# wrchen530/batrack

Hardware: AMD Instinct MI355X
Metric: BA iterations/s on 64-KF/128k-edge graph (higher is better)
Workload: dtype f32

## Files before the change

### batrack_amd/csrc/ba_plan.hpp

```cpp
#pragma once
#include <array>
#include <atomic>
#include <chrono>
#include <cstddef>
#include <cstdio>
#include <cstdint>
#include <string>
#include <vector>

#include "../../include/batrack_ba.h"

namespace bt {

constexpr int kLanes = 64;
constexpr int kTileCamSoft = 16;
constexpr int kTileCamHard = 64;
constexpr int kTileCamF64 = 32;
constexpr int kFewHubs = 64;
constexpr int kMaxFree = 255;
constexpr int kMaxFreeWide = 2048;
constexpr int kPairAccStride = 32;
constexpr int kPrivY = 16, kPrivP = 4;
constexpr int kPrivArrive = 8192;
constexpr int kPairGeomFloats = 20;
constexpr int kLdsRowStride = 66;
constexpr int kMaxLevelCols = 4;
constexpr size_t kLdsBudget = 160 * 1024 - 512;
inline size_t solve_lds_bytes_raw(size_t nnzb, size_t D, size_t nupd, size_t n, size_t nlev, size_t ndp, size_t elem) {
    size_t b = (nnzb * 36 + 2 * D) * elem;
    b = (b + 15) / 16 * 16;
    b += nupd * 3 * sizeof(unsigned short);
    b = (b + 15) / 16 * 16;
    b += (nnzb + 4 * (n + 1) + nlev + 1 + n + ndp) * sizeof(int);
    b = (b + 15) / 16 * 16 + nlev * kMaxLevelCols * 8 * sizeof(int);
    return b + 64;
}
constexpr int kSpGroupMax = 32;
constexpr int kMaxTilePairs = 192;

#ifdef __HIPCC__
#define BT_HD __host__ __device__
#else
#define BT_HD
#endif
BT_HD inline size_t priv_copy_doubles(size_t D, size_t pairs) { return (size_t)kPrivY * D + (size_t)kPrivP * pairs * kPairAccStride; }
BT_HD inline size_t priv_doubles(size_t D, size_t pairs) { return priv_copy_doubles(D, pairs) + kPrivArrive / 2; }
BT_HD inline size_t sp_tile_doubles(int max_rows16, int max_tile_pairs) {
    const size_t nt = (size_t)max_rows16 / 16;
    return nt * (nt + 1) / 2 * 256 + (size_t)max_rows16 + (size_t)(max_tile_pairs > 0 ? max_tile_pairs : 1) * 32;
}

constexpr size_t kEtileLdsBudget = 160 * 1024 - 512;
BT_HD inline size_t etile_full_lds_bytes(int max_rows16, int max_tile_pairs, size_t rsz) {
    const size_t mtp = (size_t)(max_tile_pairs > 0 ? max_tile_pairs : 1), rows = (size_t)max_rows16;
    size_t smax = 1;
    while (smax < mtp) smax <<= 1;
    return (size_t)4 * 26 * smax * sizeof(double) + (rows * kLdsRowStride + 128 + mtp * kPairGeomFloats) * rsz + rows * sizeof(int) + 64;
}

struct Route {
    enum : int { kTile = 0, kStream = 1, kEdge = 2, kEtile = 3 };
    enum : int { kSolveLds = 0, kSolveLds32 = 1, kSolveGlobal = 2, kSolveDense = 3, kSolveFused = 4, kSolvePipe = 5 };
    int kernel;
    int prec;
    int wide;
    int solver;
    int fuse_update;
    int upd_wgs;
};

struct PlanDev {
    int E, n_buf, p_tot, fixedp, n_all, n, D, m, P, T, slots, erows, nnzb, nupd, max_rows16;
    const int32_t *kx;
    const uint32_t *act_bits;
    const int32_t *act_rank;
    const int32_t *pair_i, *pair_j;
    const int32_t *tile_trk0, *tile_ntrk, *tile_ncam, *tile_cam0, *tile_slot0, *tile_nslot, *tile_erow0;
    const int32_t *tile_cams;
    const int32_t *slot_edge, *slot_pair;
    const uint16_t *slot_lab;
    const int32_t *tile_pair0, *tile_npair, *tile_pairs;
    const uint16_t *tile_cut8, *tile_cut16;
    const int32_t *tile_ij, *tile_kx;
    const int32_t *tile_flags;
    const uint8_t *slot_lp;
    int max_tile_pairs, max_tile_slots, max_cams;
    long long e_all;
    const uint16_t *slot_code;
    const uint8_t *tile_la;
    const int32_t *tile_rec;
    const int32_t *it_edge;
    const uint32_t *tile_sinfo;
    const int32_t *pm_edge, *pm_rec;
    const uint8_t *pm_lb, *pm_la;
    const int32_t *pp_ptr, *pp_idx;
    const int32_t *sg_ptr; int sg_n;
    int et_lgts;
    int sp_ok;
    int pm_ok;
    const int32_t *lz_trk, *lz_ptr, *lz_edge, *lz_pair;
    int nlz;
    int dev_id;
    int wide;
    int trk_off;
    int em_self;
    int em_ok, em_its, em_lgs;
    int st_ok;
    int st_min, em_min;
    const int32_t *col_ptr, *row_idx, *upd_ptr, *upd, *blk_col, *upd_next;
    int nlev, ndp;
    const int32_t *perm, *blk_src, *lvl_ptr, *lvl_cols, *col_lvl, *dp_ptr, *dp;
    const int32_t *fz_pend_ptr, *fz_pend, *fz_lazy_ptr, *fz_lazy, *fz_yurg, *fz_meta, *fz_pmeta, *bs_sync, *fz_rowinfo, *fz_pfirst, *fz_psecond;
    int fz_npend, fz_nlazy, fz_ok;
    int fzp_ok;
    const int32_t *lvl_meta;
    Route route;
};

constexpr size_t kStatusBytes = 1024;
constexpr int kStatusHandoff = 2;

struct WsLayout {
    size_t sys, pairacc, zero_bytes;
    size_t packed, pairgeo, qw, lfac, linv, zvec, dx, dx0, dxg, status, spart, esave, total;
    size_t priv;
};

// ... 162 lines not shown
```

### batrack_amd/csrc/ba_plan_solver.cpp

```cpp
#include "ba_plan.hpp"

#include <algorithm>
#include <numeric>

namespace bt {
namespace {

using Pattern = std::vector<std::vector<uint8_t>>;

void couple_all(Pattern &nz, std::vector<int32_t> &cset) {
    std::sort(cset.begin(), cset.end());
    cset.erase(std::unique(cset.begin(), cset.end()), cset.end());
    for (size_t u = 0; u < cset.size(); ++u)
        for (size_t v = 0; v <= u; ++v) nz[(size_t)cset[u]][(size_t)cset[v]] = 1;
}

int system_pattern(const bt_plan *pl, bool sharded, const DevPlanStats *dstats, const uint64_t *pk, int64_t E, Pattern &nz) {
    const int64_t n = pl->info.n, fixedp = pl->info.fixedp, p_tot = pl->info.p_tot;
    nz.assign((size_t)n, std::vector<uint8_t>((size_t)n, 0));
    for (int64_t c = 0; c < n; ++c) nz[(size_t)c][(size_t)c] = 1;
    for (int64_t t = 0; t < pl->info.tiles && !sharded; ++t) {
        const int32_t c0 = pl->tile_cam0[(size_t)t], nc = pl->tile_ncam[(size_t)t];
        for (int32_t u = 0; u < nc; ++u)
            for (int32_t v = 0; v <= u; ++v)
// ... 224 lines not shown
            for (int pass = 0; pass < 2; ++pass)
                for (int32_t q = pl->lvl_ptr[(size_t)l]; q < pl->lvl_ptr[(size_t)l + 1]; ++q) {
                    const int32_t j = pl->lvl_cols[(size_t)q];
                    for (int32_t b = pl->col_ptr[(size_t)j] + 1; b < pl->col_ptr[(size_t)j + 1]; ++b) {
                        const int32_t r = pl->row_idx[(size_t)b];
                        if (pass == 0) { if (seen[(size_t)r] != l) { seen[(size_t)r] = l; cnt[(size_t)r] = 0; } cnt[(size_t)r]++; }
                        else if (cnt[(size_t)r] > 1) pl->blk_col[(size_t)b] |= 1 << 16;
                    }
                }
        }
    }
    pl->dp_ptr.assign((size_t)n + 1, 0);
    pl->dp.clear();
    for (int64_t j = 0; j < n; ++j) {
        pl->dp_ptr[(size_t)j] = (int32_t)pl->dp.size();
        pl->dp.insert(pl->dp.end(), dplist[(size_t)j].begin(), dplist[(size_t)j].end());
    }
    pl->dp_ptr[(size_t)n] = (int32_t)pl->dp.size();

    pl->lvl_meta.assign((size_t)nlev * kMaxLevelCols * 8, 0);
    for (int32_t l = 0; l < nlev; ++l)
        for (int q = 0; q < kMaxLevelCols; ++q) {
            int32_t *mrow = pl->lvl_meta.data() + ((size_t)l * kMaxLevelCols + q) * 8;
            if (pl->lvl_ptr[(size_t)l] + q >= pl->lvl_ptr[(size_t)l + 1]) { mrow[0] = -1; continue; }
            const int32_t j = pl->lvl_cols[(size_t)pl->lvl_ptr[(size_t)l] + q];
            mrow[0] = j; mrow[1] = pl->col_ptr[(size_t)j]; mrow[2] = pl->col_ptr[(size_t)j + 1] - pl->col_ptr[(size_t)j] - 1;
            mrow[3] = pl->upd_ptr[(size_t)j] + pl->upd_next[(size_t)j];
            mrow[4] = pl->upd_ptr[(size_t)j + 1] - mrow[3];
            mrow[5] = pl->dp_ptr[(size_t)j]; mrow[6] = pl->dp_ptr[(size_t)j + 1] - pl->dp_ptr[(size_t)j];
            mrow[7] = pl->lvl_ptr[(size_t)l + 1] - pl->lvl_ptr[(size_t)l];
        }
}

void fused_schedule(bt_plan *pl) {
    const int64_t n = pl->info.n;
    const std::vector<int32_t> &lvl = pl->col_lvl;
    const int32_t nlev = (int32_t)pl->lvl_ptr.size() - 1;
    const size_t nb = pl->row_idx.size();
    std::vector<std::vector<int32_t>> pend(nb);
    pl->fz_lazy_ptr.assign((size_t)n + 1, 0);
    pl->fz_lazy.clear();
    pl->fz_yurg.assign(nb, 0);
    for (int64_t j = 0; j < n; ++j) {
        pl->fz_lazy_ptr[(size_t)j] = (int32_t)(pl->fz_lazy.size() / 3);
        for (int32_t t = pl->upd_ptr[(size_t)j]; t < pl->upd_ptr[(size_t)j + 1]; ++t) {
            const int32_t s1 = pl->upd[(size_t)t * 3], s2 = pl->upd[(size_t)t * 3 + 1], d = pl->upd[(size_t)t * 3 + 2];
            const int32_t dcol = pl->row_idx[(size_t)s2];
            if (lvl[(size_t)dcol] == lvl[(size_t)j] + 1) { pend[(size_t)(d & 0x7fff)].push_back(s1); pend[(size_t)(d & 0x7fff)].push_back(s2); }
            else { pl->fz_lazy.push_back(s1); pl->fz_lazy.push_back(s2); pl->fz_lazy.push_back(d); }
        }
        for (int32_t b = pl->col_ptr[(size_t)j] + 1; b < pl->col_ptr[(size_t)j + 1]; ++b)
            if (lvl[(size_t)pl->row_idx[(size_t)b]] == lvl[(size_t)j] + 1) pl->fz_yurg[(size_t)b] = 1;
    }
    pl->fz_lazy_ptr[(size_t)n] = (int32_t)(pl->fz_lazy.size() / 3);
    pl->fz_pend_ptr.assign(nb + 1, 0);
    pl->fz_pend.clear();
    for (size_t b = 0; b < nb; ++b) {
        pl->fz_pend_ptr[b] = (int32_t)(pl->fz_pend.size() / 2);
        pl->fz_pend.insert(pl->fz_pend.end(), pend[b].begin(), pend[b].end());
    }
    pl->fz_pend_ptr[nb] = (int32_t)(pl->fz_pend.size() / 2);
    pl->fz_pmeta.assign((size_t)nlev * 8, 0);
    for (int32_t l = 0; l < nlev; ++l) {
        const int32_t nc = pl->lvl_ptr[(size_t)l + 1] - pl->lvl_ptr[(size_t)l];
        int32_t *m = pl->fz_pmeta.data() + (size_t)l * 8;
        for (int32_t q = 0; q < nc && q < 2; ++q) {
            const int32_t j = pl->lvl_cols[(size_t)pl->lvl_ptr[(size_t)l] + q];
            const int32_t dpos = pl->col_ptr[(size_t)j], cnt = pl->col_ptr[(size_t)j + 1] - dpos - 1;
            const int32_t k0 = pl->fz_pend_ptr[(size_t)dpos], np = pl->fz_pend_ptr[(size_t)dpos + 1] - k0;
            const int32_t sd = np > 0 ? pl->fz_pend[(size_t)k0 * 2] : 0;
            const int32_t ysrc = np > 0 ? (pl->blk_col[(size_t)sd] & 255) : 0;
            const int32_t lz0 = pl->fz_lazy_ptr[(size_t)j], nlz = pl->fz_lazy_ptr[(size_t)j + 1] - lz0;
            m[4 * q] = j | (cnt << 8) | (ysrc << 16);
            m[4 * q + 1] = dpos | (((6 * cnt + 1 + 63) / 64) << 16);
            m[4 * q + 2] = lz0 | (nlz << 16);
            int32_t dep = 0;
            for (int32_t b = dpos; b < pl->col_ptr[(size_t)j + 1]; ++b)
                for (int32_t k = pl->fz_pend_ptr[(size_t)b]; k < pl->fz_pend_ptr[(size_t)b + 1]; ++k) {
                    const int32_t sc = pl->blk_col[(size_t)pl->fz_pend[(size_t)k * 2]] & 255;
                    for (int32_t q2 = 0; l > 0 && q2 < pl->lvl_ptr[(size_t)l] - pl->lvl_ptr[(size_t)l - 1]; ++q2)
                        if (pl->lvl_cols[(size_t)pl->lvl_ptr[(size_t)l - 1] + q2] == sc) dep |= 1 << q2;
                }
            m[4 * q + 3] = sd | ((np < 3 ? np : 3) << 15) | (dep << 20);
        }
        m[1] |= nc << 24;
    }
    pl->fz_rowinfo.assign(nb, 0);
    pl->fz_pfirst.assign(nb, 0);
    pl->fz_psecond.assign(nb, 0);
    bool pend_ok = true;
    for (size_t b = 0; b < nb; ++b) {
        pl->fz_rowinfo[b] = pl->row_idx[b] | ((pl->blk_col[b] & 255) << 8) | ((pl->blk_col[b] >> 16) << 24) | (pl->fz_yurg[b] << 25);
        const int32_t k0 = pl->fz_pend_ptr[b], c = pl->fz_pend_ptr[b + 1] - k0;
        if (c > 2) pend_ok = false;
        if (c > 0 && nb < 32768)
            pl->fz_pfirst[b] = (int32_t)((uint32_t)pl->fz_pend[(size_t)k0 * 2] | ((uint32_t)pl->fz_pend[(size_t)k0 * 2 + 1] << 15) |
                                         ((uint32_t)(c < 3 ? c : 3) << 30));
        if (c > 1 && nb < 32768)
            pl->fz_psecond[b] = (int32_t)((uint32_t)pl->fz_pend[(size_t)k0 * 2 + 2] | ((uint32_t)pl->fz_pend[(size_t)k0 * 2 + 3] << 15));
    }
    pl->bs_sync.assign((size_t)nlev, 0);
    {
        std::vector<int32_t> slot((size_t)n, 0);
        for (int32_t l = 0; l < nlev; ++l)
            for (int32_t qi = pl->lvl_ptr[(size_t)l]; qi < pl->lvl_ptr[(size_t)l + 1]; ++qi)
                slot[(size_t)pl->lvl_cols[(size_t)qi]] = qi - pl->lvl_ptr[(size_t)l];
        int32_t last_barrier = nlev;
        for (int32_t l = nlev - 1; l >= 0; --l) {
            bool need = false;
            for (int32_t qi = pl->lvl_ptr[(size_t)l]; qi < pl->lvl_ptr[(size_t)l + 1]; ++qi) {
                const int32_t j = pl->lvl_cols[(size_t)qi];
                for (int32_t b = pl->col_ptr[(size_t)j] + 1; b < pl->col_ptr[(size_t)j + 1]; ++b) {
                    const int32_t i = pl->row_idx[(size_t)b];
                    if (slot[(size_t)i] != slot[(size_t)j] && last_barrier > lvl[(size_t)i] - 1) need = true;
                }
            }
            if (need) { pl->bs_sync[(size_t)l] = 1; last_barrier = l; }
        }
    }
    pl->fz_meta.assign((size_t)nlev * kMaxLevelCols * 8, 0);
    pl->dev.fz_ok = (pl->fz_lazy.size() / 3 < 65536 && pl->row_idx.size() < 32768 && pend_ok) ? 1 : 0;
    pl->dev.fzp_ok = pl->dev.fz_ok;
    for (int64_t j = 0; j < n; ++j) if (6 * (pl->col_ptr[(size_t)j + 1] - pl->col_ptr[(size_t)j] - 1) + 1 > 64) pl->dev.fzp_ok = 0;
    for (int32_t l = 0; l < nlev; ++l) {
        if (pl->lvl_ptr[(size_t)l + 1] - pl->lvl_ptr[(size_t)l] > 2) { pl->dev.fz_ok = 0; pl->dev.fzp_ok = 0; }
        int32_t w0 = 0;
        for (int q = 0; q < kMaxLevelCols; ++q) {
            int32_t *mrow = pl->fz_meta.data() + ((size_t)l * kMaxLevelCols + q) * 8;
            if (pl->lvl_ptr[(size_t)l] + q >= pl->lvl_ptr[(size_t)l + 1]) { mrow[0] = -1; mrow[5] = w0; continue; }
            const int32_t j = pl->lvl_cols[(size_t)pl->lvl_ptr[(size_t)l] + q];
            mrow[0] = j; mrow[1] = pl->col_ptr[(size_t)j]; mrow[2] = pl->col_ptr[(size_t)j + 1] - pl->col_ptr[(size_t)j] - 1;
            mrow[3] = pl->fz_lazy_ptr[(size_t)j]; mrow[4] = pl->fz_lazy_ptr[(size_t)j + 1] - mrow[3];
            mrow[5] = w0; mrow[6] = (6 * mrow[2] + 1 + 63) / 64;
            mrow[7] = pl->lvl_ptr[(size_t)l + 1] - pl->lvl_ptr[(size_t)l];
            w0 += mrow[6];
        }
    }
}

#define BT_CLEAR_SOLVER(T, name, solver) if (solver) pl->name.clear();
void go_wide(bt_plan *pl) {
    const int64_t n = pl->info.n;
    pl->dev.wide = 1;
    BT_PLAN_TABLES(BT_CLEAR_SOLVER)
    pl->perm.resize((size_t)n);
    std::iota(pl->perm.begin(), pl->perm.end(), 0);
    pl->col_ptr.assign((size_t)n + 1, 0); pl->upd_ptr.assign((size_t)n + 1, 0); pl->upd_next.assign((size_t)n + 1, 0);
    pl->lvl_ptr.assign(1, 0); pl->dp_ptr.assign((size_t)n + 1, 0);
    pl->dev.fz_ok = 0; pl->dev.fzp_ok = 0;
    pl->info.nnz_blocks = n * (n + 1) / 2; pl->info.updates = 0;
}
#undef BT_CLEAR_SOLVER

}

int plan_reduced_system(bt_plan *pl, bool sharded, const DevPlanStats *dstats, const uint64_t *pk, int64_t E, PhaseTimer &tick) {
    const bt_plan_info &I = pl->info;
    const int64_t n = I.n;
    pl->dev.wide = 0;
    if (n > kMaxFree) { go_wide(pl); return BT_OK; }
    {
        Pattern nz;
        std::vector<int32_t> parent;
        int rc = system_pattern(pl, sharded, dstats, pk, E, nz);
        if (rc != BT_OK) return rc;
        tick("9");
// ... 19 lines not shown
```

### batrack_amd/csrc/ba_solve.hip

```cpp
#include <hip/hip_runtime.h>

#include "ba_kernels.hpp"
#include "ba_update.hpp"
#include "ba_wave.hpp"

namespace bt {

__device__ inline bool chol6_inv(float *Ablk, float *Linv) {
    float L[6][6];
#pragma unroll
    for (int r = 0; r < 6; ++r)
#pragma unroll
        for (int c = 0; c < 6; ++c) L[r][c] = c <= r ? Ablk[6*r + c] : 0.0f;
    bool ok = true;
#pragma unroll
    for (int c = 0; c < 6; ++c) {
        float s = L[c][c];
#pragma unroll
        for (int k = 0; k < c; ++k) s -= L[c][k] * L[c][k];
        if (!(s > 0.0f)) ok = false;
        const float l = sqrtf(s), il = 1.0f / l;
        L[c][c] = l;
#pragma unroll
        for (int r = c + 1; r < 6; ++r) {
// ... 52 lines not shown
            const int dpos = pd.col_ptr[j], cnt = pd.col_ptr[j + 1] - dpos - 1;
            if (tid == 0) {
                if (!chol6_inv(Lw + (size_t)dpos * 36, Li + (size_t)j * 36)) flags[0] = 1;
                float zz[6];
                for (int r = 0; r < 6; ++r) {
                    float t = 0.0f;
                    for (int c = 0; c <= r; ++c) t += Li[j*36 + 6*r + c] * z[6*j + c];
                    zz[r] = t;
                }
                for (int r = 0; r < 6; ++r) z[6*j + r] = zz[r];
            }
            __syncthreads();
            for (int idx = tid; idx < cnt * 6; idx += nth) {
                const int s = idx / 6, r = idx % 6;
                float *blk = Lw + (size_t)(dpos + 1 + s) * 36 + 6*r;
                float in[6], out[6];
                for (int c = 0; c < 6; ++c) in[c] = blk[c];
                float dot = 0.0f;
                for (int c = 0; c < 6; ++c) {
                    float t = 0.0f;
                    for (int k = 0; k <= c; ++k) t += in[k] * Li[j*36 + 6*c + k];
                    out[c] = t;
                    dot += t * z[6*j + c];
                }
                for (int c = 0; c < 6; ++c) blk[c] = out[c];
                z[6 * pd.row_idx[dpos + 1 + s] + r] -= dot;
            }
            __syncthreads();
            const int u0 = pd.upd_ptr[j], nu = pd.upd_ptr[j + 1] - u0;
            for (int idx = tid; idx < nu * 36; idx += nth) {
                const int t = idx / 36, e = idx % 36, r = e / 6, c = e % 6;
                const int *tr = pd.upd + (size_t)(u0 + t) * 3;
                const float *L1 = Lw + (size_t)tr[0] * 36 + 6*r, *L2 = Lw + (size_t)tr[1] * 36 + 6*c;
                float acc = 0.0f;
                for (int k = 0; k < 6; ++k) acc += L1[k] * L2[k];
                Lw[(size_t)(tr[2] & 0x7fff) * 36 + e] -= acc;
            }
            __syncthreads();
        }

        for (int j = n - 1; j >= 0; --j) {
            const int dpos = pd.col_ptr[j], cnt = pd.col_ptr[j + 1] - dpos - 1;
            for (int idx = tid; idx < cnt * 6; idx += nth) {
                const int s = idx / 6, c = idx % 6;
                const float *blk = Lw + (size_t)(dpos + 1 + s) * 36;
                const float *xr = z + 6 * pd.row_idx[dpos + 1 + s];
                float t = 0.0f;
                for (int r = 0; r < 6; ++r) t += blk[6*r + c] * xr[r];
                part[idx] = t;
            }
            __syncthreads();
            if (tid < 6) {
                float t = z[6*j + tid];
                for (int s = 0; s < cnt; ++s) t -= part[6*s + tid];
                tq[tid] = t;
            }
            __syncthreads();
            if (tid < 6) {
                float x = 0.0f;
                for (int r = tid; r < 6; ++r) x += Li[j*36 + 6*r + tid] * tq[r];
                z[6*j + tid] = x;
            }
            __syncthreads();
        }
        for (int i = tid; i < D; i += nth) if (z[i] != z[i]) flags[1] = 1;
        __syncthreads();
        const bool failed = flags[0] != 0, has_nan = flags[1] != 0;
        __syncthreads();
        if (failed) {
            for (int i = tid; i < D; i += nth) z[i] = 0.0f;
            status = BT_SOLVE_CHOL_FAILED;
            break;
        }
        if (!has_nan) break;
        status = BT_SOLVE_RETRIED;
    }
    __syncthreads();
    for (int i = tid; i < D; i += nth) a.dx[6 * pd.perm[i / 6] + i % 6] = z[i];
    if (tid == 0) a.status[0] = status;
}

#define BT_LT(r, c) ((r) * ((r) + 1) / 2 + (c))

template <typename T>
__device__ __forceinline__ bool chol6_packed(T (&L)[21]) {
    bool ok = true;
#pragma unroll
    for (int c = 0; c < 6; ++c) {
        T s = L[BT_LT(c, c)];
#pragma unroll
        for (int k = 0; k < c; ++k) s -= L[BT_LT(c, k)] * L[BT_LT(c, k)];
        ok = ok && (s > (T)0);
        const T il = rsqrt_t<T>(s);
        L[BT_LT(c, c)] = il;
#pragma unroll
        for (int r = c + 1; r < 6; ++r) {
            T t = L[BT_LT(r, c)];
#pragma unroll
            for (int k = 0; k < c; ++k) t -= L[BT_LT(r, k)] * L[BT_LT(c, k)];
            L[BT_LT(r, c)] = t * il;
        }
    }
    return ok;
}

template <typename T, bool RAW_DIAG>
__device__ __forceinline__ void lds_backsub_prep(T *Lw, const T *z, T *zt, const int *row_idx, const int *col_ptr, int nnzb, int tid, int nth) {
    for (int b = tid; b < nnzb; b += nth) {
        const int rc = row_idx[b], j = (rc >> 8) & 255;
        const bool diag = (rc & 255) == j;
        const T *dblk = Lw + (size_t)col_ptr[j] * 36;
        T L[21], li[21];
#pragma unroll
        for (int r = 0; r < 6; ++r) {
            T row[6];
            load_row6(dblk + 6 * r, row);
#pragma unroll
            for (int c = 0; c <= r; ++c) L[BT_LT(r, c)] = row[c];
        }
        if (RAW_DIAG) (void)chol6_packed<T>(L);
#pragma unroll
        for (int c = 0; c < 6; ++c) {
            li[BT_LT(c, c)] = L[BT_LT(c, c)];
#pragma unroll
            for (int r = c + 1; r < 6; ++r) {
                T t = (T)0;
#pragma unroll
                for (int k = c; k < r; ++k) t += L[BT_LT(r, k)] * li[BT_LT(k, c)];
                li[BT_LT(r, c)] = -t * L[BT_LT(r, r)];
            }
        }
        auto to_m = [&](const T (&in)[6], T (&out)[6]) {
#pragma unroll
            for (int c = 0; c < 6; ++c) {
                T t = li[BT_LT(c, c)] * in[c];
#pragma unroll
                for (int k = c + 1; k < 6; ++k) t += li[BT_LT(k, c)] * in[k];
                out[c] = t;
            }
        };
        if (diag) {
            T in[6], out[6];
            load_row6(z + 6 * j, in);
            to_m(in, out);
            store_row6(zt + 6 * j, out);
        } else {
            T *p = Lw + (size_t)b * 36;
            for (int h = 0; h < 3; ++h, p += 12) {
                T in[2][6], out[2][6];
#pragma unroll
                for (int u = 0; u < 2; ++u) load_row6(p + 6 * u, in[u]);
#pragma unroll
                for (int u = 0; u < 2; ++u) to_m(in[u], out[u]);
#pragma unroll
                for (int u = 0; u < 2; ++u) store_row6(p + 6 * u, out[u]);
            }
        }
    }
}

size_t solve_lds_bytes(const PlanDev &pd, size_t elem) {
    return solve_lds_bytes_raw((size_t)pd.nnzb, (size_t)pd.D, (size_t)pd.nupd, (size_t)pd.n, (size_t)pd.nlev, (size_t)pd.ndp, elem);
}

template <typename T> __device__ __forceinline__ void lds_sub(T *p, T v, bool atomic) {
    if (atomic) atomicAdd(p, -v); else *p -= v;
}

template <typename T>
__device__ __forceinline__ void apply_update_row3(T *Lw, unsigned s1, unsigned s2, unsigned d, int r) {
    T a[6], b[36], o[6], v[6];
    T *dst = Lw + (d & 0x7fffu) * 36 + 6 * r;
    const T *bb = Lw + s2 * 36;
    load_row6(Lw + s1 * 36 + 6 * r, a);
#pragma unroll
    for (int c = 0; c < 6; ++c) load_row6(bb + 6 * c, reinterpret_cast<T (&)[6]>(b[6 * c]));
    load_row6(dst, v);
    __builtin_amdgcn_sched_barrier(0);
#pragma unroll
    for (int c = 0; c < 6; ++c) {
        T acc = a[0] * b[6 * c];
#pragma unroll
        for (int k = 1; k < 6; ++k) acc += a[k] * b[6 * c + k];
        o[c] = acc;
    }
    if (d & 0x8000u) {
#pragma unroll
// ... 449 lines not shown
        A.w = word(nlev - 1);
        wn = word(nlev - 2);
        operands(A);
        for (int l = nlev - 1; l >= 0; l -= 2) {
            level(A, B, l - 2);
            level(B, A, l - 3);
        }
    } else {
        for (int l = nlev - 1; l >= 0; --l)
            if (__builtin_amdgcn_readfirstlane(tab[(kBsPad + l) * kFusedCols * 8].x) & kBsSync) __syncthreads();
    }
    __syncthreads();
}

__device__ __forceinline__ int pfirst_index(int ma, int dpos, int rw) { return rw < ((ma >> 8) & 255) * 6 ? dpos + 1 + rw / 6 : dpos; }

struct NoPoll {
    __device__ __forceinline__ void look() {}
    __device__ __forceinline__ bool passed() { return true; }
};
struct LevelPoll {
    int *colready, *hcnt;
    int need0, need1, needh, f0, f1, fh, lastfail;
    __device__ __forceinline__ void look() {
        f0 = __hip_atomic_load(&colready[0], __ATOMIC_RELAXED, __HIP_MEMORY_SCOPE_WORKGROUP);
        f1 = __hip_atomic_load(&colready[1], __ATOMIC_RELAXED, __HIP_MEMORY_SCOPE_WORKGROUP);
        fh = __hip_atomic_load(hcnt, __ATOMIC_RELAXED, __HIP_MEMORY_SCOPE_WORKGROUP);
        asm volatile("" ::: "memory");
    }
    __device__ __forceinline__ bool passed() {
        asm volatile("" ::: "memory");
        if (f0 >= need0 && f1 >= need1 && fh >= needh) {
            __builtin_amdgcn_fence(__ATOMIC_ACQUIRE, "workgroup");
            return true;
        }
        lastfail = fh < needh ? 1 : 0;
        __builtin_amdgcn_s_sleep(1);
        return false;
    }
};

template <typename T, typename Poll>
__device__ __forceinline__ T *row_wave_pending(T *Lw, T *z, const int *row_idx, unsigned pfo, const int *psecond, int ma, int dpos, int rw,
                                               bool &valid, T (&in)[6], Poll &poll) {
    const int j = ma & 255, cnt = (ma >> 8) & 255, ysrc = (ma >> 16) & 255;
    const bool isy = rw == cnt * 6;
    valid = rw <= cnt * 6;
    const int sb = rw / 6, r = rw - 6 * sb, bown = dpos + 1 + sb;
    T *p = isy ? z + 6 * j : Lw + (size_t)bown * 36 + 6 * r;
    const int s1 = pfo & 0x7fff, s2 = (pfo >> 15) & 0x7fff, no = valid ? (int)(pfo >> 30) : 0;
    T avec[6], m[36];
    const T *ap = isy ? z + 6 * ysrc : Lw + (size_t)s1 * 36 + 6 * r, *M = Lw + (size_t)(isy ? s1 : s2) * 36;
    auto look_and_load = [&]() {
        poll.look();
        load_row6(p, in);
        load_row6(ap, avec);
#pragma unroll
        for (int c = 0; c < 6; ++c) load_row6(M + 6 * c, reinterpret_cast<T (&)[6]>(m[6 * c]));
    };
    look_and_load();
    while (!poll.passed()) look_and_load();
#pragma unroll
    for (int c = 0; c < 6; ++c) {
        T acc = avec[0] * m[6 * c];
#pragma unroll
        for (int e = 1; e < 6; ++e) acc += avec[e] * m[6 * c + e];
        in[c] -= no > 0 ? acc : (T)0;
    }
    if (__builtin_amdgcn_ballot_w64(no > 1)) {
        const unsigned ps = (unsigned)psecond[isy ? dpos : bown];
        const int t1 = ps & 0x7fff, t2 = (ps >> 15) & 0x7fff;
        load_row6(isy ? z + 6 * ((row_idx[t1] >> 8) & 255) : Lw + (size_t)t1 * 36 + 6 * r, avec);
        const T *M = Lw + (size_t)(isy ? t1 : t2) * 36;
#pragma unroll
        for (int c = 0; c < 6; ++c) load_row6(M + 6 * c, reinterpret_cast<T (&)[6]>(m[6 * c]));
#pragma unroll
        for (int c = 0; c < 6; ++c) {
            T acc = avec[0] * m[6 * c];
#pragma unroll
            for (int e = 1; e < 6; ++e) acc += avec[e] * m[6 * c + e];
            in[c] -= no > 1 ? acc : (T)0;
        }
    }
    return p;
}

__host__ __device__ inline size_t sweep_work_bytes(const PlanDev &pd) {
    const size_t b = 2 * 36 * sizeof(double) +
                     (size_t)pd.fz_nlazy * 4 * sizeof(unsigned short) + 16;
    const size_t zt = (size_t)((pd.D + 1) & ~1) * sizeof(double) + backsub_table_bytes(pd);
    return ((b > zt ? b : zt) + 15) / 16 * 16;
}
size_t solve_fused_lds_bytes(const PlanDev &pd, int) {
    return ((size_t)pd.nnzb * 36 + (size_t)pd.D) * sizeof(double) + sweep_work_bytes(pd) +
           (5 * (size_t)pd.nnzb + (size_t)pd.n + 1) * sizeof(int) + 64;
}

template <bool PROF, bool PUB>
__device__ __forceinline__ void solve_fused_body(const PlanDev &pd, const StepArgs &a) {
    typedef double T;
    extern __shared__ __attribute__((aligned(16))) unsigned char smem[];
    __shared__ int flags[2];
    __shared__ int lready[kFusedCols];
    __shared__ int ntr;
    __shared__ int4 mbuf[3][2];
    const int tid = threadIdx.x, nth = blockDim.x, wave = tid >> 6, lane = tid & 63, nw = nth >> 6;
    const int n = pd.n, D = pd.D, nnzb = pd.nnzb, nlev = pd.nlev;
    T *Lw = reinterpret_cast<T *>(smem);
    T *z = Lw + (size_t)nnzb * 36, *scr = z + D, *zt = scr;
    unsigned short *lazy = reinterpret_cast<unsigned short *>(scr + kFusedCols * 36);
    int *row_idx = reinterpret_cast<int *>(reinterpret_cast<unsigned char *>(scr) + sweep_work_bytes(pd)), *pfirst = row_idx + nnzb,
        *psecond = pfirst + nnzb, *col_ptr = psecond + nnzb, *bsrc = col_ptr + n + 1, *trl = bsrc + nnzb;
    const int4 *pmeta = reinterpret_cast<const int4 *>(pd.fz_pmeta);
    for (int i = tid; i < nnzb; i += nth) { row_idx[i] = pd.fz_rowinfo[i]; pfirst[i] = pd.fz_pfirst[i]; psecond[i] = pd.fz_psecond[i]; }
    for (int i = tid; i <= n; i += nth) col_ptr[i] = pd.col_ptr[i];
    long long phA = 0, phL = 0, tph = 0, tall = PROF ? clock64() : 0, tload = 0, tsweep = 0, sub[6] = {0, 0, 0, 0, 0, 0}, tsub = 0;
#define BT_SUB(i) do { if (PROF) { asm volatile("s_waitcnt lgkmcnt(0)" ::: "memory"); const long long tq = clock64(); sub[i] += tq - tsub; tsub = tq; } } while (0)

    int status = BT_SOLVE_OK;
    for (int attempt = 0; attempt < 2; ++attempt) {
        const double lm = attempt == 0 ? 1e-4 : 1e-3;
        if (tid < 2) flags[tid] = 0;
        if (tid < kFusedCols) lready[tid] = 0;
        for (int i = tid; i < pd.fz_nlazy; i += nth)
            reinterpret_cast<ushort4 *>(lazy)[i] = make_ushort4((unsigned short)pd.fz_lazy[3 * i], (unsigned short)pd.fz_lazy[3 * i + 1],
                                                               (unsigned short)pd.fz_lazy[3 * i + 2], 0);
        if (tid < 4 && (tid >> 1) < nlev) mbuf[tid >> 1][tid & 1] = pmeta[tid];
        lds_load_system_dma<T>(pd, a, Lw, z, bsrc, trl, &ntr, col_ptr, lm, attempt == 0, true, tid, nth);
        __syncthreads();
        if (PROF) tload = clock64() - tall;

        int c0a, c0b, c0c, c0d, c1a, c1b, c1c, c1d, n0a = 0, n0b = 0, n0c = 0, n0d = 0, n1a = 0, n1b = 0, n1c = 0, n1d = 0;
        int p0a = 0, p0b = 0, p0c = 0, p1a = 0, p1b = 0, p1c = 0, pnc = 0;
        auto take_next = [&](int l) {
            const int4 m0 = mbuf[l % 3][0], m1 = mbuf[l % 3][1];
            n0a = __builtin_amdgcn_readfirstlane(m0.x); n0b = __builtin_amdgcn_readfirstlane(m0.y);
            n0c = __builtin_amdgcn_readfirstlane(m0.z); n0d = __builtin_amdgcn_readfirstlane(m0.w);
            n1a = __builtin_amdgcn_readfirstlane(m1.x); n1b = __builtin_amdgcn_readfirstlane(m1.y);
            n1c = __builtin_amdgcn_readfirstlane(m1.z); n1d = __builtin_amdgcn_readfirstlane(m1.w);
        };
        take_next(0);
        const bool feeder = tid >= nth - 2;
        for (int l = 0; l < nlev; ++l) {
            c0a = n0a; c0b = n0b; c0c = n0c; c0d = n0d; c1a = n1a; c1b = n1b; c1c = n1c; c1d = n1d;
            if (PROF) tph = clock64();
            int4 mnext = make_int4(0, 0, 0, 0);
            if (feeder && l + 2 < nlev) mnext = pmeta[(size_t)(l + 2) * 2 + (tid - (nth - 2))];
            const int cnc = (c0b >> 24) & 3;
            const int nr0 = (c0b >> 16) & 255, nr1 = cnc > 1 ? (c1b >> 16) & 255 : 0;
            const int nA = cnc + nr0 + nr1;
            for (int aw = wave; aw < nA; aw += nw) {
                __builtin_amdgcn_s_setprio(3);
                if (PROF) tsub = clock64();
                if (aw < cnc) {
                    const int q = aw, dpos = (q ? c1b : c0b) & 0xffff, md = q ? c1d : c0d;
                    const int el = lane < 36 ? lane : lane - 36, dr = el / 6, dc = el - 6 * dr;
                    const int sd = md & 0x7fff, nd = (md >> 15) & 3;
                    T x[6], yv[6];
                    T v = Lw[(size_t)dpos * 36 + el];
                    load_row6(Lw + (size_t)sd * 36 + 6 * dr, x);
                    load_row6(Lw + (size_t)sd * 36 + 6 * dc, yv);
                    if (nd > 0) {
                        T acc = x[0] * yv[0];
#pragma unroll
                        for (int e = 1; e < 6; ++e) acc += x[e] * yv[e];
                        v -= acc;
// ... 95 lines not shown
            p0a = c0a; p0b = c0b; p0c = c0c; p1a = c1a; p1b = c1b; p1c = c1c; pnc = cnc;
            if (l + 1 < nlev) take_next(l + 1);
            __syncthreads();
        }
        if (PROF) tsweep = clock64() - tall;

        int2 *btab = reinterpret_cast<int2 *>(zt + ((D + 1) & ~1));
        backsub_table(pd, btab, row_idx, tid, nth);
        long long tbs[2] = {0, 0};
        lds_back_substitute<T, true>(pd, Lw, z, zt, row_idx, col_ptr, btab, tid, nth, PROF ? tbs : nullptr);
        if (PROF) { sub[0] = tbs[0] - tall; sub[1] = tbs[1] - tall; sub[2] = clock64() - tall; }
        for (int i = tid; i < D; i += nth) if (zt[i] != zt[i]) flags[1] = 1;
        __syncthreads();
        const bool failed = flags[0] != 0, has_nan = flags[1] != 0;
        __syncthreads();
        if (failed) {
            for (int i = tid; i < D; i += nth) zt[i] = (T)0;
            status = BT_SOLVE_CHOL_FAILED;
            break;
        }
        if (!has_nan) break;
        status = BT_SOLVE_RETRIED;
    }
    __syncthreads();
    for (int i = tid; i < D; i += nth) {
        const int k = 6 * pd.perm[i / 6] + i % 6;
        a.dx[k] = (float)zt[i];
        if (PUB) dx_publish(a, k, (float)zt[i]);
    }
    if (tid == 0) a.status[0] = status;
    if (PROF && lane == 0) {
        long long *o = reinterpret_cast<long long *>(a.status + 4) + 40 + wave * 2;
        o[0] = phA; o[1] = phL;
        if (wave == 0 || wave == 2) {
            long long *g = reinterpret_cast<long long *>(a.status + 4) + (wave ? 10 : 0);
            g[0] = tload; g[1] = tsweep; g[2] = clock64() - tall;
            for (int i = 0; i < 6; ++i) g[3 + i] = sub[i];
        }
    }
#undef BT_SUB
}

template <bool PROF>
__global__ __launch_bounds__(768) void k_solve_fused(PlanDev pd, StepArgs a) { solve_fused_body<PROF, false>(pd, a); }

size_t solve_pipe_lds_bytes(const PlanDev &pd) {
    return ((size_t)pd.nnzb * 36 + (size_t)pd.D) * sizeof(double) + sweep_work_bytes(pd) +
           (5 * (size_t)pd.nnzb + (size_t)pd.n + 1 + (size_t)pd.nlev * 8) * sizeof(int) + 64;
}

__device__ __forceinline__ void wait_ge(int *flag, int target) {
    while (__hip_atomic_load(flag, __ATOMIC_RELAXED, __HIP_MEMORY_SCOPE_WORKGROUP) < target) __builtin_amdgcn_s_sleep(1);
}

template <bool PROF, bool PUB>
__device__ __forceinline__ void solve_pipe_body(const PlanDev &pd, const StepArgs &a) {
    typedef double T;
    extern __shared__ __attribute__((aligned(16))) unsigned char smem[];
    __shared__ int flags[2];
    __shared__ int lready[2], colready[2], hcnt, ntr;
    const int tid = threadIdx.x, nth = blockDim.x, wave = __builtin_amdgcn_readfirstlane(tid >> 6), lane = tid & 63, nw = nth >> 6;
    const int n = pd.n, D = pd.D, nnzb = pd.nnzb, nlev = pd.nlev;
    T *Lw = reinterpret_cast<T *>(smem);
    T *z = Lw + (size_t)nnzb * 36, *scr = z + D, *zt = scr;
    unsigned short *lazy = reinterpret_cast<unsigned short *>(scr + 2 * 36);
    int *row_idx = reinterpret_cast<int *>(reinterpret_cast<unsigned char *>(scr) + sweep_work_bytes(pd)), *pfirst = row_idx + nnzb,
        *psecond = pfirst + nnzb, *col_ptr = psecond + nnzb, *lrec = col_ptr + n + 1, *bsrc = lrec + nlev * 8, *trl = bsrc + nnzb;
    for (int i = tid; i < nnzb; i += nth) { row_idx[i] = pd.fz_rowinfo[i]; pfirst[i] = pd.fz_pfirst[i]; psecond[i] = pd.fz_psecond[i]; }
    for (int i = tid; i <= n; i += nth) col_ptr[i] = pd.col_ptr[i];
    for (int i = tid; i < nlev * 8; i += nth) lrec[i] = pd.fz_pmeta[i];
    long long tall = PROF ? clock64() : 0, tload = 0, tsweep = 0, twait = 0, twork = 0, tq = 0, sub[3] = {0, 0, 0}, wsplit[2] = {0, 0};
#define BT_TW(acc) do { if (PROF) { asm volatile("s_waitcnt lgkmcnt(0)" ::: "memory"); const long long tn = clock64(); acc += tn - tq; tq = tn; } } while (0)

    int status = BT_SOLVE_OK;
    for (int attempt = 0; attempt < 2; ++attempt) {
        const double lm = attempt == 0 ? 1e-4 : 1e-3;
        if (tid < 2) { flags[tid] = 0; lready[tid] = 0; colready[tid] = 0; }
        if (tid == 2) hcnt = 0;
        int nlazy = pd.fz_nlazy;
        asm volatile("" : "+s"(nlazy));
        for (int i = tid; i < nlazy; i += nth)
            reinterpret_cast<ushort4 *>(lazy)[i] = make_ushort4((unsigned short)pd.fz_lazy[3 * i], (unsigned short)pd.fz_lazy[3 * i + 1],
                                                               (unsigned short)pd.fz_lazy[3 * i + 2], 0);
        lds_load_system_dma<T>(pd, a, Lw, z, bsrc, trl, &ntr, col_ptr, lm, attempt == 0, true, tid, nth);
        __syncthreads();
        if (PROF) { tload = clock64() - tall; tq = clock64(); }

        const int nh = nw - 4;
        if (wave < 4) {
            const int q = wave & 1;
            const bool is_row = wave >= 2;
            const int4 *lrec4 = reinterpret_cast<const int4 *>(lrec);
            int4 vrec = lrec4[q];
            int vnc = lrec[1];
            int npc = 0;
            unsigned pfn = is_row ? (unsigned)pfirst[pfirst_index(vrec.x, vrec.y & 0xffff, lane)] : 0u;
            for (int l = 0; l < nlev; ++l) {
                const int ma = __builtin_amdgcn_readfirstlane(vrec.x), mb = __builtin_amdgcn_readfirstlane(vrec.y),
                          md = __builtin_amdgcn_readfirstlane(vrec.w), ncl = (__builtin_amdgcn_readfirstlane(vnc) >> 24) & 3;
                auto next_record = [&]() { if (l + 1 < nlev) { vrec = lrec4[2 * (l + 1) + q]; vnc = lrec[8 * (l + 1) + 1]; } };
                if (!is_row) next_record();
                if (q < ncl) {
                    const int dep = l > 0 ? ((md >> 20) & 3) | ((!is_row && q < npc) ? 1 << q : 0) : 0;
                    LevelPoll poll = {colready, &hcnt, (dep & 1) ? l : 0, (dep & 2) ? l : 0, l > 0 ? nh * (l - 1) : 0, 0, 0, 0, -1};
                    const long long tw0 = PROF ? clock64() : 0;
                    const int dpos = mb & 0xffff;
                    if (!is_row) {
                        const int el = lane < 36 ? lane : lane - 36, dr = el / 6, dc = el - 6 * dr;
                        const int sd = md & 0x7fff, nd = (md >> 15) & 3;
                        T x[6], yv[6];
                        T v;
                        do poll.look(); while (!poll.passed());
                        v = Lw[(size_t)dpos * 36 + el];
                        load_row6(Lw + (size_t)sd * 36 + 6 * dr, x);
                        load_row6(Lw + (size_t)sd * 36 + 6 * dc, yv);
                        if (PROF && poll.lastfail >= 0) wsplit[poll.lastfail] += clock64() - tw0;
                        BT_TW(twait);
                        if (nd > 0) {
                            T acc = x[0] * yv[0];
#pragma unroll
                            for (int e = 1; e < 6; ++e) acc += x[e] * yv[e];
                            v -= acc;
                        }
                        if (nd > 1) {
                            const T *src = Lw + (size_t)(psecond[dpos] & 0x7fff) * 36;
                            load_row6(src + 6 * dr, x);
                            load_row6(src + 6 * dc, yv);
                            T acc = x[0] * yv[0];
#pragma unroll
                            for (int e = 1; e < 6; ++e) acc += x[e] * yv[e];
                            v -= acc;
                        }
                        if (lane < 36) {
                            scr[q * 36 + lane] = v;
                            Lw[(size_t)dpos * 36 + lane] = v;
                        }
                        __builtin_amdgcn_fence(__ATOMIC_RELEASE, "workgroup");
                        if (lane == 0) __hip_atomic_store(&lready[q], l + 1, __ATOMIC_RELAXED, __HIP_MEMORY_SCOPE_WORKGROUP);
                        BT_TW(twork);
                    } else {
                        bool valid;
                        T in[6];
                        T *p = row_wave_pending(Lw, z, row_idx, pfn, psecond, ma, dpos, lane, valid, in, poll);
                        if (PROF && poll.lastfail >= 0) wsplit[poll.lastfail] += clock64() - tw0;
                        BT_TW(sub[0]);
                        T L[21];
                        int lrf;
                        auto look_and_load = [&]() {
                            lrf = __hip_atomic_load(&lready[q], __ATOMIC_RELAXED, __HIP_MEMORY_SCOPE_WORKGROUP);
                            asm volatile("" ::: "memory");
                            const T *dblk = scr + q * 36;
#pragma unroll
                            for (int rr = 0; rr < 6; ++rr) {
                                T row[6];
                                load_row6(dblk + 6 * rr, row);
#pragma unroll
                                for (int c = 0; c <= rr; ++c) L[BT_LT(rr, c)] = row[c];
                            }
                            next_record();
                            asm volatile("" ::: "memory");
                        };
                        look_and_load();
                        while (lrf <= l) { __builtin_amdgcn_s_sleep(1); look_and_load(); }
                        __builtin_amdgcn_fence(__ATOMIC_ACQUIRE, "workgroup");
                        if (l + 1 < nlev) pfn = (unsigned)pfirst[pfirst_index(vrec.x, vrec.y & 0xffff, lane)];
                        BT_TW(sub[1]);
                        const bool ok = chol6_packed<T>(L);
                        T out[6];
#pragma unroll
                        for (int c = 0; c < 6; ++c) {
                            T t = in[c];
#pragma unroll
                            for (int k = 0; k < c; ++k) t -= out[k] * L[BT_LT(c, k)];
                            out[c] = t * L[BT_LT(c, c)];
                        }
                        if (valid) store_row6(p, out);
                        if (!ok && lane == 0) flags[0] = 1;
                        __builtin_amdgcn_fence(__ATOMIC_RELEASE, "workgroup");
                        if (lane == 0) __hip_atomic_store(&colready[q], l + 1, __ATOMIC_RELAXED, __HIP_MEMORY_SCOPE_WORKGROUP);
                        BT_TW(sub[2]);
                    }
                } else if (is_row && l + 1 < nlev) {
                    next_record();
                    pfn = (unsigned)pfirst[pfirst_index(vrec.x, vrec.y & 0xffff, lane)];
                    asm volatile("s_waitcnt lgkmcnt(0)" : "+v"(pfn));
                }
                npc = ncl;
            }
        } else {
            const int h = tid - 256, hs = nth - 256;
            for (int b = 0; b + 1 < nlev; ++b) {
                const int p0a = __builtin_amdgcn_readfirstlane(lrec[8 * b]), p0b = __builtin_amdgcn_readfirstlane(lrec[8 * b + 1]),
                          p0c = __builtin_amdgcn_readfirstlane(lrec[8 * b + 2]), p1a = __builtin_amdgcn_readfirstlane(lrec[8 * b + 4]),
                          p1b = __builtin_amdgcn_readfirstlane(lrec[8 * b + 5]), p1c = __builtin_amdgcn_readfirstlane(lrec[8 * b + 6]);
                const int pnc = (p0b >> 24) & 3;
                {
                    const int need1 = pnc > 1 ? b + 1 : 0;
                    for (;;) {
                        const int f0 = __hip_atomic_load(&colready[0], __ATOMIC_RELAXED, __HIP_MEMORY_SCOPE_WORKGROUP);
                        const int f1 = __hip_atomic_load(&colready[1], __ATOMIC_RELAXED, __HIP_MEMORY_SCOPE_WORKGROUP);
                        const int fh = __hip_atomic_load(&hcnt, __ATOMIC_RELAXED, __HIP_MEMORY_SCOPE_WORKGROUP);
                        if (f0 >= b + 1 && f1 >= need1 && fh >= nh * b) break;
                        __builtin_amdgcn_s_sleep(1);
                    }
                }
                __builtin_amdgcn_fence(__ATOMIC_ACQUIRE, "workgroup");
                BT_TW(twait);
                const int rows0 = ((p0c >> 16) & 0xffff) * 6, rows1 = rows0 + (pnc > 1 ? ((p1c >> 16) & 0xffff) * 6 : 0);
                for (int item = h; item < rows1; item += hs) {
                    const bool sec = item >= rows0;
                    const int idx = item - (sec ? rows0 : 0), t = idx / 6;
                    const ushort4 tr = reinterpret_cast<const ushort4 *>(lazy)[((sec ? p1c : p0c) & 0xffff) + t];
                    apply_update_row3<T>(Lw, tr.x, tr.y, tr.z, idx - 6 * t);
                }
                {
                    const int ys0 = ((p0a >> 8) & 255) * 6, ys1 = ys0 + (pnc > 1 ? ((p1a >> 8) & 255) * 6 : 0);
                    const int shift = ((rows1 + 63) >> 6) << 6;
                    int first = h - shift;
                    if (shift > hs) first = (h - shift % hs + hs) % hs; else if (first < 0) first += hs;
                    for (int item = first; item < ys1; item += hs) {
                        const bool sec = item >= ys0;
                        const int qq = item - (sec ? ys0 : 0);
                        const int pj = (sec ? p1a : p0a) & 255, dposp = (sec ? p1b : p0b) & 0xffff, sb = qq / 6, r = qq - 6 * sb;
                        const int rcv = row_idx[dposp + 1 + sb];
                        if (rcv & (1 << 25)) continue;
                        T lr[6], zr[6];
                        load_row6(Lw + (size_t)(dposp + 1 + sb) * 36 + 6 * r, lr);
                        load_row6(z + 6 * pj, zr);
                        T acc = lr[0] * zr[0];
#pragma unroll
                        for (int k = 1; k < 6; ++k) acc += lr[k] * zr[k];
                        lds_sub(z + 6 * (rcv & 255) + r, acc, (rcv & (1 << 24)) != 0);
                    }
                }
                __builtin_amdgcn_fence(__ATOMIC_RELEASE, "workgroup");
                if (lane == 0) __hip_atomic_fetch_add(&hcnt, 1, __ATOMIC_RELAXED, __HIP_MEMORY_SCOPE_WORKGROUP);
                BT_TW(twork);
            }
        }
        __syncthreads();
        if (PROF) tsweep = clock64() - tall;

        int2 *btab = reinterpret_cast<int2 *>(zt + ((D + 1) & ~1));
        backsub_table(pd, btab, row_idx, tid, nth);
        lds_back_substitute<T, true>(pd, Lw, z, zt, row_idx, col_ptr, btab, tid, nth, nullptr);
        for (int i = tid; i < D; i += nth) if (zt[i] != zt[i]) flags[1] = 1;
        __syncthreads();
        const bool failed = flags[0] != 0, has_nan = flags[1] != 0;
        __syncthreads();
        if (failed) {
            for (int i = tid; i < D; i += nth) zt[i] = (T)0;
            status = BT_SOLVE_CHOL_FAILED;
            break;
        }
        if (!has_nan) break;
        status = BT_SOLVE_RETRIED;
    }
    __syncthreads();
    for (int i = tid; i < D; i += nth) {
        const int k = 6 * pd.perm[i / 6] + i % 6;
        a.dx[k] = (float)zt[i];
        if (PUB) dx_publish(a, k, (float)zt[i]);
    }
    if (tid == 0) a.status[0] = status;
    if (PROF && lane == 0) {
        long long *o = reinterpret_cast<long long *>(a.status + 4) + 40 + wave * 2;
        o[0] = twait; o[1] = twork + sub[0] + sub[2];
// ... 83 lines not shown
```

Before: 13300.

## Keep chained-column Cholesky updates in registers via cross-lane readlane instead of LDS handoff

The planner now tags levels whose column depends only on the previous level's single column in a simple chained pattern. For these levels the row wave keeps the previous column's factored rows in registers, applies the pending update with readlane broadcasts, and factors the diagonal block itself. This skips the LDS publish/poll handoff with the diagonal wave. Row-to-lane assignment is rotated per level so each level's diagonal rows land in a known lane group. The cost is more register pressure and more complex lane mapping, and it is limited to double precision in the reg path.

```diff
diff --git a/batrack_amd/csrc/ba_plan.hpp b/batrack_amd/csrc/ba_plan.hpp
--- a/batrack_amd/csrc/ba_plan.hpp
+++ b/batrack_amd/csrc/ba_plan.hpp
@@ -43,6 +43,8 @@
 #else
 #define BT_HD
 #endif
+constexpr int kRegLaneGroups = 8;
+BT_HD inline int pipe_lane_group(int l, int k) { return (l + 1 + k) & (kRegLaneGroups - 1); }
 BT_HD inline size_t priv_copy_doubles(size_t D, size_t pairs) { return (size_t)kPrivY * D + (size_t)kPrivP * pairs * kPairAccStride; }
 BT_HD inline size_t priv_doubles(size_t D, size_t pairs) { return priv_copy_doubles(D, pairs) + kPrivArrive / 2; }
 BT_HD inline size_t sp_tile_doubles(int max_rows16, int max_tile_pairs) {
diff --git a/batrack_amd/csrc/ba_plan_solver.cpp b/batrack_amd/csrc/ba_plan_solver.cpp
--- a/batrack_amd/csrc/ba_plan_solver.cpp
+++ b/batrack_amd/csrc/ba_plan_solver.cpp
@@ -330,6 +330,17 @@
                         if (pl->lvl_cols[(size_t)pl->lvl_ptr[(size_t)l - 1] + q2] == sc) dep |= 1 << q2;
                 }
             m[4 * q + 3] = sd | ((np < 3 ? np : 3) << 15) | (dep << 20);
+            if (l > 0 && q < pl->lvl_ptr[(size_t)l] - pl->lvl_ptr[(size_t)l - 1]) {
+                const int32_t jp = pl->lvl_cols[(size_t)pl->lvl_ptr[(size_t)l - 1] + q];
+                const int32_t dp = pl->col_ptr[(size_t)jp], cp = pl->col_ptr[(size_t)jp + 1] - dp - 1;
+                bool reg = cnt < kRegLaneGroups && cp < kRegLaneGroups && cp >= 1 && cnt >= cp - 1 && pl->row_idx[(size_t)dp + 1] == j &&
+                           np == 1 && sd == dp + 1 && pl->fz_pend[(size_t)k0 * 2 + 1] == dp + 1 && dep == 1 << q;
+                for (int32_t k = 0; k < cnt && reg; ++k) {
+                    const int32_t kk = pl->fz_pend_ptr[(size_t)dpos + 1 + k], c = pl->fz_pend_ptr[(size_t)dpos + 2 + k] - kk;
+                    reg = k < cp - 1 ? c == 1 && pl->fz_pend[(size_t)kk * 2] == dp + 2 + k && pl->fz_pend[(size_t)kk * 2 + 1] == dp + 1 : c == 0;
+                }
+                if (reg) m[4 * q + 3] |= 1 << 22 | pipe_lane_group(l, -1) << 23;
+            }
         }
         m[1] |= nc << 24;
     }
diff --git a/batrack_amd/csrc/ba_solve.hip b/batrack_amd/csrc/ba_solve.hip
--- a/batrack_amd/csrc/ba_solve.hip
+++ b/batrack_amd/csrc/ba_solve.hip
@@ -158,14 +158,15 @@
 
 #define BT_LT(r, c) ((r) * ((r) + 1) / 2 + (c))
 
-template <typename T>
-__device__ __forceinline__ bool chol6_packed(T (&L)[21]) {
+template <typename T, typename Fetch>
+__device__ __forceinline__ bool chol6_packed(T (&L)[21], Fetch fetch) {
     bool ok = true;
 #pragma unroll
     for (int c = 0; c < 6; ++c) {
         T s = L[BT_LT(c, c)];
 #pragma unroll
         for (int k = 0; k < c; ++k) s -= L[BT_LT(c, k)] * L[BT_LT(c, k)];
+        fetch(c, s);
         ok = ok && (s > (T)0);
         const T il = rsqrt_t<T>(s);
         L[BT_LT(c, c)] = il;
@@ -179,6 +180,8 @@
     }
     return ok;
 }
+template <typename T>
+__device__ __forceinline__ bool chol6_packed(T (&L)[21]) { return chol6_packed(L, [](int, T &) {}); }
 
 template <typename T, bool RAW_DIAG>
 __device__ __forceinline__ void lds_backsub_prep(T *Lw, const T *z, T *zt, const int *row_idx, const int *col_ptr, int nnzb, int tid, int nth) {
@@ -794,6 +797,48 @@
             in[c] -= no > 1 ? acc : (T)0;
         }
     }
+    return p;
+}
+
+__device__ __forceinline__ int pipe_row_of_lane(int ma, int l, int lane) {
+    const int cnt = (ma >> 8) & 255, g = lane / 6, sb = (g - pipe_lane_group(l, 0)) & (kRegLaneGroups - 1);
+    if (cnt >= kRegLaneGroups) return lane;
+    return lane == 6 * kRegLaneGroups ? 6 * cnt : lane < 6 * kRegLaneGroups && sb < cnt ? 6 * sb + (lane - 6 * g) : 6 * cnt + 1;
+}
+__device__ __forceinline__ double readlane_f64(double v, int srclane) {
+    return __hiloint2double(__builtin_amdgcn_readlane(__double2hiint(v), srclane), __builtin_amdgcn_readlane(__double2loint(v), srclane));
+}
+
+constexpr bool kRegDiag = true;
+
+template <typename Poll>
+__device__ __forceinline__ double *row_wave_pending_reg(double *Lw, double *z, unsigned pfo, int ma, int dpos, int rw, int lane, int g,
+                                                        const double (&prev)[6], bool &valid, bool &diag, double (&in)[6], Poll &poll) {
+    const int j = ma & 255, cnt = (ma >> 8) & 255;
+    const bool isy = rw == cnt * 6;
+    valid = rw <= cnt * 6;
+    diag = kRegDiag && lane / 6 == g;
+    const int sb = rw / 6, r = rw - 6 * sb;
+    double *p = isy ? z + 6 * j : diag ? Lw + (size_t)dpos * 36 + 6 * (lane - 6 * g) : Lw + (size_t)(dpos + 1 + sb) * 36 + 6 * r;
+    const int no = valid || diag ? (int)(pfo >> 30) : 0;
+    poll.look();
+    load_row6(p, in);
+    double a[6], acc[6];
+#pragma unroll
+    for (int e = 0; e < 6; ++e) a[e] = prev[e];
+#pragma unroll
+    for (int e = 0; e < 6; ++e) {
+        if (e > 0) asm volatile("" : "+v"(a[e]), "+v"(acc[0]), "+v"(acc[1]), "+v"(acc[2]), "+v"(acc[3]), "+v"(acc[4]), "+v"(acc[5]));
+#pragma unroll
+        for (int c = 0; c < 6; ++c) {
+            const double m = readlane_f64(a[e], 6 * g + c);
+            acc[c] = e == 0 ? a[0] * m : acc[c] + a[e] * m;
+        }
+    }
+    asm volatile("" : "+v"(acc[0]), "+v"(acc[1]), "+v"(acc[2]), "+v"(acc[3]), "+v"(acc[4]), "+v"(acc[5]));
+    while (!poll.passed()) { poll.look(); load_row6(p, in); }
+#pragma unroll
+    for (int c = 0; c < 6; ++c) in[c] -= no > 0 ? acc[c] : 0.0;
     return p;
 }
 
@@ -1055,7 +1100,9 @@
         for (int i = tid; i < nlazy; i += nth)
             reinterpret_cast<ushort4 *>(lazy)[i] = make_ushort4((unsigned short)pd.fz_lazy[3 * i], (unsigned short)pd.fz_lazy[3 * i + 1],
                                                                (unsigned short)pd.fz_lazy[3 * i + 2], 0);
-        lds_load_system_dma<T>(pd, a, Lw, z, bsrc, trl, &ntr, col_ptr, lm, attempt == 0, true, tid, nth);
+        int ltid = tid;
+        asm volatile("" : "+v"(ltid));
+        lds_load_system_dma<T>(pd, a, Lw, z, bsrc, trl, &ntr, col_ptr, lm, attempt == 0, true, ltid, nth);
         __syncthreads();
         if (PROF) { tload = clock64() - tall; tq = clock64(); }
 
@@ -1067,7 +1114,10 @@
             int4 vrec = lrec4[q];
             int vnc = lrec[1];
             int npc = 0;
-            unsigned pfn = is_row ? (unsigned)pfirst[pfirst_index(vrec.x, vrec.y & 0xffff, lane)] : 0u;
+            int rlane = lane;
+            asm volatile("" : "+v"(rlane));
+            unsigned pfn = is_row ? (unsigned)pfirst[pfirst_index(vrec.x, vrec.y & 0xffff, pipe_row_of_lane(vrec.x, 0, rlane))] : 0u;
+            T out[6] = {};
             for (int l = 0; l < nlev; ++l) {
                 const int ma = __builtin_amdgcn_readfirstlane(vrec.x), mb = __builtin_amdgcn_readfirstlane(vrec.y),
                           md = __builtin_amdgcn_readfirstlane(vrec.w), ncl = (__builtin_amdgcn_readfirstlane(vnc) >> 24) & 3;
@@ -1078,7 +1128,9 @@
                     LevelPoll poll = {colready, &hcnt, (dep & 1) ? l : 0, (dep & 2) ? l : 0, l > 0 ? nh * (l - 1) : 0, 0, 0, 0, -1};
                     const long long tw0 = PROF ? clock64() : 0;
                     const int dpos = mb & 0xffff;
-                    if (!is_row) {
+                    const bool reg = (md >> 22) & 1;
+                    if (!is_row && kRegDiag && reg) {
+                    } else if (!is_row) {
                         const int el = lane < 36 ? lane : lane - 36, dr = el / 6, dc = el - 6 * dr;
                         const int sd = md & 0x7fff, nd = (md >> 15) & 3;
                         T x[6], yv[6];
@@ -1112,40 +1164,71 @@
                         if (lane == 0) __hip_atomic_store(&lready[q], l + 1, __ATOMIC_RELAXED, __HIP_MEMORY_SCOPE_WORKGROUP);
                         BT_TW(twork);
                     } else {
-                        bool valid;
+                        bool valid, diag = false;
                         T in[6];
-                        T *p = row_wave_pending(Lw, z, row_idx, pfn, psecond, ma, dpos, lane, valid, in, poll);
-                        if (PROF && poll.lastfail >= 0) wsplit[poll.lastfail] += clock64() - tw0;
-                        BT_TW(sub[0]);
+                        T *p;
                         T L[21];
-                        int lrf;
-                        auto look_and_load = [&]() {
-                            lrf = __hip_atomic_load(&lready[q], __ATOMIC_RELAXED, __HIP_MEMORY_SCOPE_WORKGROUP);
-                            asm volatile("" ::: "memory");
-                            const T *dblk = scr + q * 36;
-#pragma unroll
-                            for (int rr = 0; rr < 6; ++rr) {
-                                T row[6];
-                                load_row6(dblk + 6 * rr, row);
-#pragma unroll
-                                for (int c = 0; c <= rr; ++c) L[BT_LT(rr, c)] = row[c];
+                        auto published_block = [&]() {
+                            int lrf;
+                            auto look_and_load = [&]() {
+                                lrf = __hip_atomic_load(&lready[q], __ATOMIC_RELAXED, __HIP_MEMORY_SCOPE_WORKGROUP);
+                                asm volatile("" ::: "memory");
+                                const T *dblk = scr + q * 36;
+#pragma unroll
+                                for (int rr = 0; rr < 6; ++rr) {
+                                    T row[6];
+                                    load_row6(dblk + 6 * rr, row);
+#pragma unroll
+                                    for (int c = 0; c <= rr; ++c) L[BT_LT(rr, c)] = row[c];
+                                }
+                                next_record();
+                                asm volatile("" ::: "memory");
+                            };
+                            look_and_load();
+                            while (lrf <= l) { __builtin_amdgcn_s_sleep(1); look_and_load(); }
+                            __builtin_amdgcn_fence(__ATOMIC_ACQUIRE, "workgroup");
+                        };
+                        auto factor_and_substitute = [&](auto fetch) {
+                            const bool fine = chol6_packed(L, fetch);
+#pragma unroll
+                            for (int c = 0; c < 6; ++c) {
+                                T t = in[c];
+#pragma unroll
+                                for (int k = 0; k < c; ++k) t -= out[k] * L[BT_LT(c, k)];
+                                out[c] = t * L[BT_LT(c, c)];
                             }
+                            return fine;
+                        };
+                        auto next_pfirst = [&]() {
+                            if (l + 1 < nlev) pfn = (unsigned)pfirst[pfirst_index(vrec.x, vrec.y & 0xffff, pipe_row_of_lane(vrec.x, l + 1, rlane))];
+                        };
+                        const int rg = (md >> 23) & (kRegLaneGroups - 1);
+                        bool ok;
+                        if (kRegDiag && reg) {
+                            p = row_wave_pending_reg(Lw, z, pfn, ma, dpos, pipe_row_of_lane(ma, l, rlane), rlane, rg, out, valid, diag, in, poll);
+                            if (PROF && poll.lastfail >= 0) wsplit[poll.lastfail] += clock64() - tw0;
+                            BT_TW(sub[0]);
                             next_record();
-                            asm volatile("" ::: "memory");
-                        };
-                        look_and_load();
-                        while (lrf <= l) { __builtin_amdgcn_s_sleep(1); look_and_load(); }
-                        __builtin_amdgcn_fence(__ATOMIC_ACQUIRE, "workgroup");
-                        if (l + 1 < nlev) pfn = (unsigned)pfirst[pfirst_index(vrec.x, vrec.y & 0xffff, lane)];
-                        BT_TW(sub[1]);
-                        const bool ok = chol6_packed<T>(L);
-                        T out[6];
-#pragma unroll
-                        for (int c = 0; c < 6; ++c) {
-                            T t = in[c];
-#pragma unroll
-                            for (int k = 0; k < c; ++k) t -= out[k] * L[BT_LT(c, k)];
-                            out[c] = t * L[BT_LT(c, c)];
+                            if (diag) store_row6(p, in);
+                            auto diag_column = [&](int c) {
+#pragma unroll
+                                for (int r = c; r < 6; ++r) L[BT_LT(r, c)] = readlane_f64(in[c], 6 * rg + r);
+                            };
+                            diag_column(0);
+                            next_pfirst();
+                            BT_TW(sub[1]);
+                            ok = factor_and_substitute([&](int c, T &s) {
+                                if (c < 5) { asm volatile("" : "+v"(s), "+v"(in[c + 1])); diag_column(c + 1); }
+                            });
+                        } else {
+                            if (reg) p = row_wave_pending_reg(Lw, z, pfn, ma, dpos, pipe_row_of_lane(ma, l, rlane), rlane, rg, out, valid, diag, in, poll);
+                            else p = row_wave_pending(Lw, z, row_idx, pfn, psecond, ma, dpos, pipe_row_of_lane(ma, l, rlane), valid, in, poll);
+                            if (PROF && poll.lastfail >= 0) wsplit[poll.lastfail] += clock64() - tw0;
+                            BT_TW(sub[0]);
+                            published_block();
+                            next_pfirst();
+                            BT_TW(sub[1]);
+                            ok = factor_and_substitute([](int, T &) {});
                         }
                         if (valid) store_row6(p, out);
                         if (!ok && lane == 0) flags[0] = 1;
@@ -1155,7 +1238,7 @@
                     }
                 } else if (is_row && l + 1 < nlev) {
                     next_record();
-                    pfn = (unsigned)pfirst[pfirst_index(vrec.x, vrec.y & 0xffff, lane)];
+                    pfn = (unsigned)pfirst[pfirst_index(vrec.x, vrec.y & 0xffff, pipe_row_of_lane(vrec.x, l + 1, rlane))];
                     asm volatile("s_waitcnt lgkmcnt(0)" : "+v"(pfn));
                 }
                 npc = ncl;
```

Measured after the change: 10830. 18.6% lower.
